# zdebruine/RcppML

Measured on AMD Instinct MI355X. Metric: ALS updates/sec (cols solved/s), k=64 sparse NMF, higher is better.
Workload: dtype f32; 1 GPU; configs[1]: simulateNMF 20000x100000 (x1 GPUs, column shards) 1%-dense CSC, k=64, MSE, coordinate-descent NNLS (cd_maxit=100, cd_tol=1e-8), L1 row normalisation, loss every iteration; rows=20000, cols_per_gpu=100000, nnz_per_gpu=20054852, k=64, solver=cd, cd_variant=auto, parallelism=column-shard x1

## Files before the change

rcppml_amd/csrc/kernels.hip.h:

```cpp
#pragma once
#include <hip/hip_runtime.h>
#include <stdint.h>

namespace rk {

#define RK_WAVE_SYNC()                                              \
    do {                                                            \
        __builtin_amdgcn_fence(__ATOMIC_RELEASE, "wavefront");      \
        __builtin_amdgcn_wave_barrier();                            \
        __builtin_amdgcn_fence(__ATOMIC_ACQUIRE, "wavefront");      \
    } while (0)

typedef float f32x4 __attribute__((ext_vector_type(4)));
typedef float f32x16 __attribute__((ext_vector_type(16)));
typedef double f64x4 __attribute__((ext_vector_type(4)));
typedef double f64x2 __attribute__((ext_vector_type(2)));

__device__ __forceinline__ float tabs(float v) { return __builtin_fabsf(v); }
__device__ __forceinline__ double tabs(double v) { return __builtin_fabs(v); }
__device__ __forceinline__ float tfma(float a, float b, float c) { return __builtin_fmaf(a, b, c); }
__device__ __forceinline__ double tfma(double a, double b, double c) { return __builtin_fma(a, b, c); }

__device__ __forceinline__ float sweep_quotient(float b, float , float ginv) { return b * ginv; }
__device__ __forceinline__ double sweep_quotient(double b, double gd, double ) { return b / gd; }
__device__ __forceinline__ double cd_quotient(double b, double gd, double ginv) {
    const double q0 = b * ginv;
    return __builtin_fma(__builtin_fma(-q0, gd, b), ginv, q0);
}
__device__ __forceinline__ float cd_quotient(float b, float , float ginv) { return b * ginv; }
__device__ __forceinline__ float cd_static_diff(float b, float , float ginv, float nl1) { return __builtin_fmaf(b, ginv, nl1); }
__device__ __forceinline__ double cd_static_diff(double b, double gd, double ginv, double nl1) { return cd_quotient(b, gd, ginv) + nl1; }
__device__ __forceinline__ float lane_value(float v, int i) {
    return __uint_as_float(__builtin_amdgcn_readlane(__float_as_uint(v), i));
}
__device__ __forceinline__ double lane_value(double v, int i) {
    const unsigned long long u = __double_as_longlong(v);
    const unsigned lo = __builtin_amdgcn_readlane((unsigned)u, i), hi = __builtin_amdgcn_readlane((unsigned)(u >> 32), i);
    return __longlong_as_double(((unsigned long long)hi << 32) | lo);
}

template <int B, int E, class Fn> __device__ __forceinline__ void cd_static_for(Fn&& fn) {
    if constexpr (B < E) { fn(std::integral_constant<int, B>{}); cd_static_for<B + 1, E>(fn); }
}
template <int I> __device__ __forceinline__ float cd_write_lane(float v, float value) {
    asm volatile("s_nop 1\n\tv_writelane_b32 %0, %1, %2" : "+v"(v) : "s"(value), "n"(I));
    return v;
}
template <int I> __device__ __forceinline__ double cd_write_lane(double v, double value) {
    unsigned long long u = __double_as_longlong(v);
    const unsigned long long w = __double_as_longlong(value);
    unsigned lo = (unsigned)u, hi = (unsigned)(u >> 32);
    asm volatile("s_nop 1\n\tv_writelane_b32 %0, %2, %4\n\tv_writelane_b32 %1, %3, %4" : "+v"(lo), "+v"(hi) : "s"((unsigned)w), "s"((unsigned)(w >> 32)), "n"(I));
    return __longlong_as_double(((unsigned long long)hi << 32) | lo);
}
__device__ __forceinline__ float cd_static_max(float a, float b, float inf) { return __builtin_amdgcn_fmed3f(a, b, inf); }
__device__ __forceinline__ double cd_static_max(double a, double b, double) { return __builtin_fmax(a, b); }
template <class T, int KP, class GC>
__device__ __forceinline__ T cd_static_one_sweep(T& b, T xe, T gd, T ginv, T nl1, T inf_rt, GC&& gcol) {
    T aown = T(0);
    cd_static_for<0, KP>([&](auto IC) {
        constexpr int i = decltype(IC)::value;
        const T diff = cd_static_diff(b, gd, ginv, nl1);
        const T ad = cd_static_max(diff, -xe, inf_rt);
        const T ad_i = lane_value(ad, i);
        b = tfma(-gcol(IC), ad_i, b);
        aown = cd_write_lane<i>(aown, ad_i);
    });
    return aown;
}
template <class T, int KP, class GC>
__device__ __forceinline__ int cd_static_sweeps(T& b, T& x, T gd, bool fok, T l1, int nonneg, int maxit, GC&& gcol) {
    const bool alive = fok && gd > T(0);
    const T ginv = alive ? T(1) / gd : T(0);
    const T nl1 = alive ? -l1 : T(0);
    const T pinf = static_cast<T>(__builtin_inff());
    const T inf_rt = maxit >= 0 ? pinf : T(0);
    for (int it = 0; it < maxit; ++it) {
        const T xe = !alive ? T(0) : (nonneg ? x : pinf);
        const T aown = cd_static_one_sweep<T, KP>(b, xe, gd, ginv, nl1, inf_rt, gcol);
        const T xn = x + aown;
        const bool moved = xn != x;
        x = xn;
        if (!__any(moved)) return it + 1;
    }
    return maxit > 0 ? maxit : 0;
}
template <class T, int KP, class GC>
__device__ __forceinline__ int cd_static_sweeps_tol(T& b, T& x, T gd, bool fok, int nonneg, int maxit, T tol, int k, GC&& gcol) {
    const bool alive = fok && gd > T(0);
    const T ginv = alive ? T(1) / gd : T(0);
    const T pinf = static_cast<T>(__builtin_inff());
    const T inf_rt = maxit >= 0 ? pinf : T(0);
    const bool check = tol > T(0);
    const T inv_k = T(1) / static_cast<T>(k);
    for (int it = 0; it < maxit; ++it) {
        const T xe = !alive ? T(0) : (nonneg ? x : pinf);
        const T aown = cd_static_one_sweep<T, KP>(b, xe, gd, ginv, T(0), inf_rt, gcol);
        const T xn = x + aown;
        const bool moved = xn != x;
        x = xn;
        if (check) {
            T term = fok ? (aown < T(0) ? -aown : aown) / ((x < T(0) ? -x : x) + T(1e-15)) : T(0);
#pragma unroll
            for (int off = 32; off > 0; off >>= 1) term += __shfl_xor(term, off, 64);
            if (term * inv_k < tol) return it + 1;
        } else if (!__any(moved)) return maxit;
    }
    return maxit;
}
template <int KP>
__device__ __forceinline__ int cd_static_sweeps_scaled_f32(float b, float& x, float gd, bool fok, float l1, int nonneg, int maxit,
                                                           float (&gcol)[KP]) {
    const bool alive = fok && gd > 0.f;
    const float ginv = alive ? 1.f / gd : 0.f;
    const float pinf = __builtin_inff();
    const float inf_rt = maxit >= 0 ? pinf : 0.f;
#pragma unroll
    for (int i = 0; i < KP; ++i) gcol[i] *= ginv;
    float d = __builtin_fmaf(b, ginv, alive ? -l1 : 0.f);
    for (int it = 0; it < maxit; ++it) {
        const float xe = nonneg ? x : pinf;
        float aown = 0.f;
        cd_static_for<0, KP>([&](auto IC) {
            constexpr int i = decltype(IC)::value;
            const float ad = cd_static_max(d, -xe, inf_rt);
            const float ad_i = lane_value(ad, i);
            d = __builtin_fmaf(-gcol[i], ad_i, d);
            aown = cd_write_lane<i>(aown, ad_i);
        });
        const float xn = x + aown;
        const bool moved = xn != x;
        x = xn;
        if (!__any(moved)) return it + 1;
    }
    return maxit > 0 ? maxit : 0;
}
template <int KP, class GC>
__device__ __forceinline__ int cd_static_sweeps_f32(float& b, float& x, float gd, bool fok, float l1, int nonneg, int maxit, GC&& gcol) {
    return cd_static_sweeps<float, KP>(b, x, gd, fok, l1, nonneg, maxit, gcol);
}

__device__ __forceinline__ float shfl_xor_t(float v, int m) { return __shfl_xor(v, m, 64); }
__device__ __forceinline__ double shfl_xor_t(double v, int m) { return __shfl_xor(v, m, 64); }

template <class T, int VEC> struct VecT;
template <> struct VecT<float, 1> { typedef float type; };
template <> struct VecT<float, 2> { typedef float type __attribute__((ext_vector_type(2))); };
template <> struct VecT<float, 4> { typedef float type __attribute__((ext_vector_type(4))); };
template <> struct VecT<double, 1> { typedef double type; };
template <> struct VecT<double, 2> { typedef double type __attribute__((ext_vector_type(2))); };

template <int T_TILES, bool VL, int STEPS>
__global__ __launch_bounds__(256) void gram_partial_f32(const float* __restrict__ F, int k, int64_t r,
                                                         float* __restrict__ partial) {
    constexpr int KP = 32 * T_TILES;
    __shared__ float red[3][T_TILES * 1024];
    const int ti = blockIdx.y;
    const int wave = threadIdx.x >> 6, lane = threadIdx.x & 63;
    const int64_t nw = (int64_t)gridDim.x * 4, wid = (int64_t)blockIdx.x * 4 + wave;
    const int64_t npairs = (r + 1) / 2;
    const int64_t per = (npairs + nw - 1) / nw;
    const int64_t p0 = wid * per;
    const int64_t p1 = p0 + per < npairs ? p0 + per : npairs;
    const int kk = lane >> 5, row = lane & 31;
    f32x16 acc[T_TILES];
#pragma unroll
    for (int t = 0; t < T_TILES; ++t)
#pragma unroll
        for (int v = 0; v < 16; ++v) acc[t][v] = 0.f;
    for (int64_t pb = p0; pb < p1; pb += STEPS) {
        float a[STEPS][T_TILES];
#pragma unroll
        for (int s = 0; s < STEPS; ++s) {
            const int64_t c = 2 * (pb + s) + kk;
            const bool cok = (pb + s) < p1 && c < r;
            const float* fc = F + c * (int64_t)k;
            if constexpr (VL) {
                typedef typename VecT<float, T_TILES>::type V;
                const int r0 = T_TILES * row;
                if (cok && r0 < k) {
                    const V v = *reinterpret_cast<const V*>(fc + r0);
#pragma unroll
                    for (int t = 0; t < T_TILES; ++t) a[s][t] = v[t];
                } else {
#pragma unroll
                    for (int t = 0; t < T_TILES; ++t) a[s][t] = 0.f;
                }
            } else {
#pragma unroll
                for (int t = 0; t < T_TILES; ++t) {
                    const int rr = 32 * t + row;
                    a[s][t] = (cok && rr < k) ? fc[rr] : 0.f;
                }
            }
        }
#pragma unroll
        for (int s = 0; s < STEPS; ++s)
#pragma unroll
            for (int t = 0; t < T_TILES; ++t) {
                float ai = a[s][0];
#pragma unroll
                for (int t2 = 1; t2 < T_TILES; ++t2) ai = (ti == t2) ? a[s][t2] : ai;
                acc[t] = __builtin_amdgcn_mfma_f32_32x32x2f32(ai, a[s][t], acc[t], 0, 0, 0);
            }
    }
    if (wave > 0) {
#pragma unroll
        for (int t = 0; t < T_TILES; ++t)
#pragma unroll
            for (int v = 0; v < 16; ++v) red[wave - 1][t * 1024 + v * 64 + lane] = acc[t][v];
    }
    __syncthreads();
    if (wave == 0) {
        float* out = partial + ((int64_t)blockIdx.x * KP * KP);
#pragma unroll
        for (int t = 0; t < T_TILES; ++t)
#pragma unroll
            for (int v = 0; v < 16; ++v) {
                float s = acc[t][v];
                s += red[0][t * 1024 + v * 64 + lane];
                s += red[1][t * 1024 + v * 64 + lane];
                s += red[2][t * 1024 + v * 64 + lane];
                const int is = (v & 3) + 8 * (v >> 2) + 4 * (lane >> 5), js = lane & 31;
                const int i = VL ? T_TILES * is + ti : 32 * ti + is;
                const int j = VL ? T_TILES * js + t : 32 * t + js;
                out[(int64_t)j * KP + i] = s;
            }
    }
}

template <int STEPS, bool SCALE>
__device__ __forceinline__ void gram_partial_f32_k64_body(float* __restrict__ F, int k, int64_t r, float* __restrict__ partial,
                                                          const unsigned bid, const unsigned nb, const float* __restrict__ sums,
                                                          int norm_type) {
    constexpr int KP = 64;
    __shared__ float red[3][4 * 1024];
    const int wave = threadIdx.x >> 6, lane = threadIdx.x & 63;
    const int64_t nw = (int64_t)nb * 4, wid = (int64_t)bid * 4 + wave;
    const int64_t npairs = (r + 1) / 2;
    const int64_t per = (npairs + nw - 1) / nw;
    const int64_t p0 = wid * per;
    const int64_t p1 = p0 + per < npairs ? p0 + per : npairs;
    const int kk = lane >> 5, row = lane & 31;
    f32x16 acc[2][2];
#pragma unroll
    for (int a = 0; a < 2; ++a)
#pragma unroll
        for (int b = 0; b < 2; ++b)
#pragma unroll
            for (int v = 0; v < 16; ++v) acc[a][b][v] = 0.f;
    typedef VecT<float, 2>::type V;
    float dv0 = 1.f, dv1 = 1.f;
    if constexpr (SCALE) {
        if (2 * row < k) {
            float s0 = sums[2 * row], s1 = sums[2 * row + 1];
            if (norm_type == 1) { s0 = sqrtf(s0); s1 = sqrtf(s1); }
            dv0 = s0 + 1e-15f; dv1 = s1 + 1e-15f;
        }
    }
    for (int64_t pb = p0; pb < p1; pb += STEPS) {
        float a[STEPS][2];
#pragma unroll
        for (int s = 0; s < STEPS; ++s) {
            const int64_t c = 2 * (pb + s) + kk;
            const bool cok = (pb + s) < p1 && c < r;
            const int r0 = 2 * row;
            if (cok && r0 < k) {
                V v = *reinterpret_cast<const V*>(F + c * (int64_t)k + r0);
                if constexpr (SCALE) {
                    v[0] = v[0] / dv0; v[1] = v[1] / dv1;
                    *reinterpret_cast<V*>(F + c * (int64_t)k + r0) = v;
                }
                a[s][0] = v[0]; a[s][1] = v[1];
            } else { a[s][0] = 0.f; a[s][1] = 0.f; }
        }
#pragma unroll
        for (int s = 0; s < STEPS; ++s)
#pragma unroll
            for (int ti = 0; ti < 2; ++ti)
#pragma unroll
                for (int t = 0; t < 2; ++t)
                    acc[ti][t] = __builtin_amdgcn_mfma_f32_32x32x2f32(a[s][ti], a[s][t], acc[ti][t], 0, 0, 0);
    }
    if (wave > 0) {
#pragma unroll
        for (int ti = 0; ti < 2; ++ti)
#pragma unroll
            for (int t = 0; t < 2; ++t)
#pragma unroll
                for (int v = 0; v < 16; ++v) red[wave - 1][(ti * 2 + t) * 1024 + v * 64 + lane] = acc[ti][t][v];
    }
    __syncthreads();
    if (wave == 0) {
        float* out = partial + ((int64_t)bid * KP * KP);
#pragma unroll
        for (int ti = 0; ti < 2; ++ti)
#pragma unroll
            for (int t = 0; t < 2; ++t)
#pragma unroll
                for (int v = 0; v < 16; ++v) {
                    float s = acc[ti][t][v];
                    s += red[0][(ti * 2 + t) * 1024 + v * 64 + lane];
                    s += red[1][(ti * 2 + t) * 1024 + v * 64 + lane];
                    s += red[2][(ti * 2 + t) * 1024 + v * 64 + lane];
                    const int is = (v & 3) + 8 * (v >> 2) + 4 * (lane >> 5), js = lane & 31;
                    out[(int64_t)(2 * js + t) * KP + (2 * is + ti)] = s;
                }
    }
}
template <int STEPS>
__global__ __launch_bounds__(256) void gram_partial_f32_k64(const float* __restrict__ F, int k, int64_t r,
                                                             float* __restrict__ partial) {
    gram_partial_f32_k64_body<STEPS, false>(const_cast<float*>(F), k, r, partial, blockIdx.x, gridDim.x, nullptr, 0);
}

template <int T_TILES>
__global__ __launch_bounds__(256) void gram_partial_f64(const double* __restrict__ F, int k, int64_t r,
                                                         double* __restrict__ partial) {
    constexpr int KP = 16 * T_TILES;
    __shared__ double red[3][T_TILES * 256];
    const int ti = blockIdx.y;
    const int wave = threadIdx.x >> 6, lane = threadIdx.x & 63;
    const int64_t nw = (int64_t)gridDim.x * 4, wid = (int64_t)blockIdx.x * 4 + wave;
    const int64_t nquad = (r + 3) / 4;
    const int64_t per = (nquad + nw - 1) / nw;
    const int64_t p0 = wid * per;
    const int64_t p1 = p0 + per < nquad ? p0 + per : nquad;
    const int kk = lane >> 4, row = lane & 15;
    f64x4 acc[T_TILES];
#pragma unroll
    for (int t = 0; t < T_TILES; ++t)
#pragma unroll
        for (int v = 0; v < 4; ++v) acc[t][v] = 0.0;
    const int rowi = 16 * ti + row;
#pragma unroll 2
    for (int64_t p = p0; p < p1; ++p) {
        const int64_t c = 4 * p + kk;
        const bool cok = c < r;
        const double* fc = F + c * (int64_t)k;
        const double ai = (cok && rowi < k) ? fc[rowi] : 0.0;
        double a[T_TILES];
#pragma unroll
        for (int t = 0; t < T_TILES; ++t) {
            const int rr = 16 * t + row;
            a[t] = (cok && rr < k) ? fc[rr] : 0.0;
        }
#pragma unroll
        for (int t = 0; t < T_TILES; ++t)
            acc[t] = __builtin_amdgcn_mfma_f64_16x16x4f64(ai, a[t], acc[t], 0, 0, 0);
    }
    if (wave > 0) {
#pragma unroll
        for (int t = 0; t < T_TILES; ++t)
#pragma unroll
            for (int v = 0; v < 4; ++v) red[wave - 1][t * 256 + v * 64 + lane] = acc[t][v];
    }
    __syncthreads();
    if (wave == 0) {
        double* out = partial + ((int64_t)blockIdx.x * KP * KP);
#pragma unroll
        for (int t = 0; t < T_TILES; ++t)
#pragma unroll
            for (int v = 0; v < 4; ++v) {
                double s = acc[t][v];
                s += red[0][t * 256 + v * 64 + lane];
                s += red[1][t * 256 + v * 64 + lane];
                s += red[2][t * 256 + v * 64 + lane];
                const int i = 16 * ti + (lane >> 4) + 4 * v;
                const int j = 16 * t + (lane & 15);
                out[(int64_t)j * KP + i] = s;
            }
    }
}

template <class T>
__device__ __forceinline__ void gram_finalize_body(const T* __restrict__ partial, int nblk, int KP, int k, T eps, T l2,
                                                   T* __restrict__ G, const unsigned bid) {
    const int e = bid * 8 + (threadIdx.x >> 5);
    const int sl = threadIdx.x & 31;
    T s = 0;
    if (e < KP * KP)
        for (int b = sl; b < nblk; b += 32) s += partial[(int64_t)b * KP * KP + e];
#pragma unroll
    for (int off = 16; off > 0; off >>= 1) s += shfl_xor_t(s, off);
    if (e >= KP * KP || sl != 0) return;
    const int i = e % KP, j = e / KP;
    if (i >= k || j >= k) return;
    if (i == j) { s += eps; s += l2; }
    G[(int64_t)j * k + i] = s;
}
template <class T>
__global__ __launch_bounds__(256) void gram_finalize(const T* __restrict__ partial, int nblk, int KP, int k, T eps, T l2,
                                                      T* __restrict__ G) {
    gram_finalize_body<T>(partial, nblk, KP, k, eps, l2, G, blockIdx.x);
}

template <class T, int VEC, int LPN, int U, bool NT>
__global__ __launch_bounds__(256) void rhs_kernel(const int* __restrict__ colptr,
                                                   const int* __restrict__ rowidx,
                                                   const T* __restrict__ vals, int64_t ncols,
                                                   const T* __restrict__ F, int k,
                                                   T* __restrict__ B) {
    constexpr int NG = 64 / LPN;
    const int64_t j = (int64_t)blockIdx.x * 4 + (threadIdx.x >> 6);
    if (j >= ncols) return;
    const int lane = threadIdx.x & 63;
    const int g = lane / LPN, li = lane % LPN;
    const int f0 = li * VEC;
    const bool fok = f0 < k;
    const int start = colptr[j], end = colptr[j + 1];
    T acc[VEC];
#pragma unroll
    for (int e = 0; e < VEC; ++e) acc[e] = T(0);
    const T* Fl = F + f0;
    for (int t = start + g; t < end; t += NG * U) {
        int rr[U];
        T vv[U];
#pragma unroll
        for (int u = 0; u < U; ++u) {
            const int tt = t + u * NG;
            const bool ok = tt < end;
            rr[u] = ok ? rowidx[tt] : 0;
            vv[u] = ok ? vals[tt] : T(0);
        }
        T ff[U][VEC];
#pragma unroll
        for (int u = 0; u < U; ++u) {
            if (fok) {
                const T* src = Fl + (int64_t)rr[u] * k;
                if constexpr (VEC == 1) {
                    ff[u][0] = src[0];
                } else {
                    typedef typename VecT<T, VEC>::type V;
                    V v;
                    if constexpr (NT) v = __builtin_nontemporal_load(reinterpret_cast<const V*>(src));
                    else v = *reinterpret_cast<const V*>(src);
#pragma unroll
                    for (int e = 0; e < VEC; ++e) ff[u][e] = v[e];
                }
            } else {
#pragma unroll
                for (int e = 0; e < VEC; ++e) ff[u][e] = T(0);
            }
        }
#pragma unroll
        for (int u = 0; u < U; ++u)
#pragma unroll
            for (int e = 0; e < VEC; ++e) acc[e] = tfma(vv[u], ff[u][e], acc[e]);
    }
#pragma unroll
    for (int off = LPN; off < 64; off <<= 1)
#pragma unroll
        for (int e = 0; e < VEC; ++e) acc[e] += shfl_xor_t(acc[e], off);
    if (g == 0 && fok) {
        T* dst = B + j * (int64_t)k + f0;
        if constexpr (VEC == 1) {
            dst[0] = acc[0];
        } else {
            typedef typename VecT<T, VEC>::type V;
            V v;
#pragma unroll
            for (int e = 0; e < VEC; ++e) v[e] = acc[e];
            *reinterpret_cast<V*>(dst) = v;
        }
    }
}

template <class T, int EPL>
__global__ __launch_bounds__(256) void rhs_generic_kernel(const int* __restrict__ colptr, const int* __restrict__ rowidx,
                                                           const T* __restrict__ vals, int64_t ncols,
                                                           const T* __restrict__ F, int k, T* __restrict__ B) {
    const int64_t j = (int64_t)blockIdx.x * 4 + (threadIdx.x >> 6);
    if (j >= ncols) return;
    const int lane = threadIdx.x & 63;
    T acc[EPL];
#pragma unroll
    for (int e = 0; e < EPL; ++e) acc[e] = T(0);
    const int start = colptr[j], end = colptr[j + 1];
#pragma unroll 4
    for (int t = start; t < end; ++t) {
        const int row = rowidx[t];
        const T v = vals[t];
        const T* src = F + (int64_t)row * k;
#pragma unroll
        for (int e = 0; e < EPL; ++e) {
            const int f = lane + 64 * e;
            if (f < k) acc[e] = tfma(v, src[f], acc[e]);
        }
    }
#pragma unroll
    for (int e = 0; e < EPL; ++e) {
        const int f = lane + 64 * e;
        if (f < k) B[j * (int64_t)k + f] = acc[e];
    }
}

template <class T, int VEC, int LPN, int U>
__global__ __launch_bounds__(256) void rhs_stage_kernel(const int* __restrict__ colptr,
                                                         const int* __restrict__ rowidx,
                                                         const T* __restrict__ vals, int64_t ncols,
                                                         const T* __restrict__ F, int k,
                                                         T* __restrict__ B) {
    constexpr int NG = 64 / LPN;
    constexpr int CH = NG * U;
    static_assert(CH <= 64, "one lane per staged nonzero");
    const int64_t j = (int64_t)blockIdx.x * 4 + (threadIdx.x >> 6);
    if (j >= ncols) return;
    const int lane = threadIdx.x & 63;
    const int g = lane / LPN, li = lane % LPN;
    const int f0 = li * VEC;
    const bool fok = f0 < k;
    const int start = colptr[j], end = colptr[j + 1];
    T acc[VEC];
#pragma unroll
    for (int e = 0; e < VEC; ++e) acc[e] = T(0);
    const T* Fl = F + (fok ? f0 : 0);
    int ri_n = 0;
    T vi_n = T(0);
    if (start < end) {
        const int tt = start + lane;
        const int tc = tt < end ? tt : end - 1;
        const int r0 = rowidx[tc];
        const T v0 = vals[tc];
        const bool ok = lane < CH && tt < end;
        ri_n = ok ? r0 : 0;
        vi_n = ok ? v0 : T(0);
    }
    for (int t0 = start; t0 < end; t0 += CH) {
        const int ri = ri_n;
        const T vi = vi_n;
        {
            const int tt = t0 + CH + lane;
            const int tc = tt < end ? tt : end - 1;
            const int r0 = rowidx[tc];
            const T v0 = vals[tc];
            __builtin_amdgcn_sched_barrier(0);
            const bool ok = lane < CH && tt < end;
            ri_n = ok ? r0 : 0;
            vi_n = ok ? v0 : T(0);
        }
        T ff[U][VEC];
        T vv[U];
#pragma unroll
        for (int u = 0; u < U; ++u) {
            const int nz = u * NG + g;
            const int r = __shfl(ri, nz, 64);
            vv[u] = __shfl(vi, nz, 64);
            const T* src = Fl + (int64_t)r * k;
            if constexpr (VEC == 1) {
                ff[u][0] = src[0];
            } else {
                typedef typename VecT<T, VEC>::type V;
                const V v = *reinterpret_cast<const V*>(src);
#pragma unroll
                for (int e = 0; e < VEC; ++e) ff[u][e] = v[e];
            }
        }
#pragma unroll
        for (int u = 0; u < U; ++u)
#pragma unroll
            for (int e = 0; e < VEC; ++e) acc[e] = tfma(vv[u], ff[u][e], acc[e]);
    }
#pragma unroll
    for (int off = LPN; off < 64; off <<= 1)
#pragma unroll
        for (int e = 0; e < VEC; ++e) acc[e] += shfl_xor_t(acc[e], off);
    if (g == 0 && fok) {
        T* dst = B + j * (int64_t)k + f0;
        if constexpr (VEC == 1) {
            dst[0] = acc[0];
        } else {
            typedef typename VecT<T, VEC>::type V;
            V v;
#pragma unroll
            for (int e = 0; e < VEC; ++e) v[e] = acc[e];
            *reinterpret_cast<V*>(dst) = v;
        }
    }
}

template <class T, int EPL, int U>
__global__ __launch_bounds__(256) void rhs_wave_kernel(const int* __restrict__ colptr,
                                                        const int* __restrict__ rowidx,
                                                        const T* __restrict__ vals, int64_t ncols,
                                                        const T* __restrict__ F, int k, T* __restrict__ B) {
    const int64_t j = __builtin_amdgcn_readfirstlane((int)((int64_t)blockIdx.x * 4 + (threadIdx.x >> 6)));
    if (j >= ncols) return;
    const int lane = threadIdx.x & 63;
    const bool fok = lane * EPL < k;
    const int f0 = fok ? lane * EPL : 0;
    const int start = colptr[j], end = colptr[j + 1];
    T acc[EPL];
#pragma unroll
    for (int e = 0; e < EPL; ++e) acc[e] = T(0);
    const T* Fl = F + f0;
    auto gather_fma = [&](const int (&rr)[U], const T (&vv)[U]) {
        T ff[U][EPL];
#pragma unroll
        for (int u = 0; u < U; ++u) {
            const T* src = Fl + (int64_t)rr[u] * k;
            if constexpr (EPL == 1) ff[u][0] = src[0];
            else {
                typedef typename VecT<T, EPL>::type V;
                const V v = *reinterpret_cast<const V*>(src);
#pragma unroll
                for (int e = 0; e < EPL; ++e) ff[u][e] = v[e];
            }
        }
#pragma unroll
        for (int u = 0; u < U; ++u)
#pragma unroll
            for (int e = 0; e < EPL; ++e) acc[e] = tfma(vv[u], ff[u][e], acc[e]);
    };
    struct __attribute__((packed, aligned(4))) IdxPack { int v[U]; };
// ... 1118 lines not shown
```

rcppml_amd/csrc/kernels_tail.hip.h:

```cpp
#pragma once
#include "kernels.hip.h"

namespace rk {

template <class T, int VEC>
__global__ __launch_bounds__(256) void tail_norm_hist_kernel(const T* __restrict__ X, int k, int64_t ncols, int norm_type,
                                                              T* __restrict__ partial, unsigned nb_norm, const int* __restrict__ sweeps,
                                                              unsigned int* __restrict__ part, unsigned nb_order) {
    if (blockIdx.x < nb_order) { order_hist_body(sweeps, ncols, part, blockIdx.x, nb_order); return; }
    const unsigned bid = blockIdx.x - nb_order;
    if constexpr (VEC > 0) row_norm_partial_vec_body<T, VEC>(X, k, ncols, norm_type, partial, bid, nb_norm);
    else row_norm_partial_body<T>(X, k, ncols, norm_type, partial, bid, nb_norm);
}
template <class T, int VEC>
__global__ __launch_bounds__(256) void tail_scale_scatter_kernel(T* __restrict__ X, int k, int64_t total, const T* __restrict__ sums,
                                                                  int norm_type, T* __restrict__ d, unsigned nb_scale,
                                                                  const int* __restrict__ sweeps, int64_t ncols,
                                                                  const unsigned int* __restrict__ part, int* __restrict__ order,
                                                                  unsigned nb_order) {
    if (blockIdx.x < nb_order) { order_scatter_body(sweeps, ncols, part, order, blockIdx.x, nb_order); return; }
    const unsigned bid = blockIdx.x - nb_order;
    if constexpr (VEC > 0) scale_rows_from_sums_vec_body<T, VEC>(X, k, total, sums, norm_type, d, bid, nb_scale);
    else scale_rows_from_sums_body<T>(X, k, total, sums, norm_type, d, bid, nb_scale);
}
template <int STEPS>
__global__ __launch_bounds__(256) void tail_scale_gram_k64_kernel(float* __restrict__ X, int k, int64_t ncols, const float* __restrict__ sums,
                                                                   int norm_type, float* __restrict__ d, float* __restrict__ gpartial,
                                                                   unsigned nb_gram, const int* __restrict__ sweeps,
                                                                   const unsigned int* __restrict__ part, int* __restrict__ order,
                                                                   unsigned nb_order) {
    if (blockIdx.x < nb_order) { order_scatter_body(sweeps, ncols, part, order, blockIdx.x, nb_order); return; }
    const unsigned bid = blockIdx.x - nb_order;
    if (bid == 0)
        for (int f = threadIdx.x; f < k; f += blockDim.x) {
            float s = sums[f];
            if (norm_type == 1) s = sqrtf(s);
            d[f] = s + 1e-15f;
        }
    gram_partial_f32_k64_body<STEPS, true>(X, k, ncols, gpartial, bid, nb_gram, sums, norm_type);
}
template <class T>
__global__ __launch_bounds__(256) void tail_gramfin_cross_kernel(const T* __restrict__ gpartial, int nblk_g, int KP, int k, T eps, T l2,
                                                                  T* __restrict__ G, const T* __restrict__ W, const T* __restrict__ Bw,
                                                                  const T* __restrict__ d, int64_t total, double* __restrict__ cpartial,
                                                                  unsigned nb_cross) {
    __shared__ double sh[4];
    if (blockIdx.x < nb_cross) cross_partial_body<T>(W, Bw, d, k, total, cpartial, blockIdx.x, nb_cross, sh);
    else gram_finalize_body<T>(gpartial, nblk_g, KP, k, eps, l2, G, blockIdx.x - nb_cross);
}

}
```

Before: 112.0 million cols/s.

## Software-pipeline k64 Gram partial loads with multi-stage register prefetch

```diff
diff --git a/rcppml_amd/csrc/kernels.hip.h b/rcppml_amd/csrc/kernels.hip.h
--- a/rcppml_amd/csrc/kernels.hip.h
+++ b/rcppml_amd/csrc/kernels.hip.h
@@ -235,7 +235,7 @@
                                                           int norm_type) {
     constexpr int KP = 64;
     __shared__ float red[3][4 * 1024];
-    const int wave = threadIdx.x >> 6, lane = threadIdx.x & 63;
+    const int wave = __builtin_amdgcn_readfirstlane((int)(threadIdx.x >> 6)), lane = threadIdx.x & 63;
     const int64_t nw = (int64_t)nb * 4, wid = (int64_t)bid * 4 + wave;
     const int64_t npairs = (r + 1) / 2;
     const int64_t per = (npairs + nw - 1) / nw;
@@ -250,37 +250,81 @@
 #pragma unroll
             for (int v = 0; v < 16; ++v) acc[a][b][v] = 0.f;
     typedef VecT<float, 2>::type V;
+    constexpr int DEPTH = 4;
+    const int r0 = 2 * row;
+    const bool rok = r0 < k;
+    const unsigned loff = (unsigned)(kk * k + r0);
+    int64_t pf = p1 > p0 ? p0 + (p1 - p0) / STEPS * STEPS : p0;
+    if (pf > p0 && 2 * pf > r) pf -= STEPS;
+    auto in_range = [&](const int64_t p) { return rok && p < p1 && 2 * p + kk < r; };
+    auto load_full = [&](V (&b)[STEPS], const int64_t pb) {
+#pragma unroll
+        for (int s = 0; s < STEPS; ++s) { b[s][0] = 0.f; b[s][1] = 0.f; }
+        if (rok) {
+#pragma unroll
+            for (int s = 0; s < STEPS; ++s) b[s] = *reinterpret_cast<const V*>(F + 2 * (pb + s) * (int64_t)k + loff);
+        }
+    };
+    auto mma_round = [&](const V (&v)[STEPS]) {
+#pragma unroll
+        for (int s = 0; s < STEPS; ++s)
+#pragma unroll
+            for (int ti = 0; ti < 2; ++ti)
+#pragma unroll
+                for (int t = 0; t < 2; ++t)
+                    acc[ti][t] = __builtin_amdgcn_mfma_f32_32x32x2f32(v[s][ti], v[s][t], acc[ti][t], 0, 0, 0);
+    };
+    V buf[DEPTH][STEPS], rag[STEPS];
+#pragma unroll
+    for (int j = 0; j < DEPTH; ++j)
+        if (p0 + j * STEPS < pf) load_full(buf[j], p0 + j * STEPS);
+    if (pf < p1) {
+#pragma unroll
+        for (int s = 0; s < STEPS; ++s) {
+            rag[s][0] = 0.f; rag[s][1] = 0.f;
+            if (in_range(pf + s)) rag[s] = *reinterpret_cast<const V*>(F + 2 * (pf + s) * (int64_t)k + loff);
+        }
+    }
     float dv0 = 1.f, dv1 = 1.f;
     if constexpr (SCALE) {
-        if (2 * row < k) {
+        if (rok) {
             float s0 = sums[2 * row], s1 = sums[2 * row + 1];
             if (norm_type == 1) { s0 = sqrtf(s0); s1 = sqrtf(s1); }
             dv0 = s0 + 1e-15f; dv1 = s1 + 1e-15f;
         }
     }
-    for (int64_t pb = p0; pb < p1; pb += STEPS) {
-        float a[STEPS][2];
-#pragma unroll
-        for (int s = 0; s < STEPS; ++s) {
-            const int64_t c = 2 * (pb + s) + kk;
-            const bool cok = (pb + s) < p1 && c < r;
-            const int r0 = 2 * row;
-            if (cok && r0 < k) {
-                V v = *reinterpret_cast<const V*>(F + c * (int64_t)k + r0);
+    for (int64_t pg = p0; pg < pf; pg += DEPTH * STEPS) {
+#pragma unroll
+        for (int j = 0; j < DEPTH; ++j) {
+            const int64_t pb = pg + j * STEPS;
+            if (pb < pf) {
+                V v[STEPS];
+#pragma unroll
+                for (int s = 0; s < STEPS; ++s) v[s] = buf[j][s];
+                if (pb + DEPTH * STEPS < pf) load_full(buf[j], pb + DEPTH * STEPS);
                 if constexpr (SCALE) {
-                    v[0] = v[0] / dv0; v[1] = v[1] / dv1;
-                    *reinterpret_cast<V*>(F + c * (int64_t)k + r0) = v;
+                    if (rok) {
+#pragma unroll
+                        for (int s = 0; s < STEPS; ++s) {
+                            v[s][0] = v[s][0] / dv0; v[s][1] = v[s][1] / dv1;
+                            *reinterpret_cast<V*>(F + 2 * (pb + s) * (int64_t)k + loff) = v[s];
+                        }
+                    }
                 }
-                a[s][0] = v[0]; a[s][1] = v[1];
-            } else { a[s][0] = 0.f; a[s][1] = 0.f; }
-        }
-#pragma unroll
-        for (int s = 0; s < STEPS; ++s)
-#pragma unroll
-            for (int ti = 0; ti < 2; ++ti)
-#pragma unroll
-                for (int t = 0; t < 2; ++t)
-                    acc[ti][t] = __builtin_amdgcn_mfma_f32_32x32x2f32(a[s][ti], a[s][t], acc[ti][t], 0, 0, 0);
+                mma_round(v);
+            }
+        }
+    }
+    if (pf < p1) {
+        if constexpr (SCALE) {
+#pragma unroll
+            for (int s = 0; s < STEPS; ++s)
+                if (in_range(pf + s)) {
+                    rag[s][0] = rag[s][0] / dv0; rag[s][1] = rag[s][1] / dv1;
+                    *reinterpret_cast<V*>(F + 2 * (pf + s) * (int64_t)k + loff) = rag[s];
+                }
+        }
+        mma_round(rag);
     }
     if (wave > 0) {
 #pragma unroll
@@ -309,7 +353,7 @@
     }
 }
 template <int STEPS>
-__global__ __launch_bounds__(256) void gram_partial_f32_k64(const float* __restrict__ F, int k, int64_t r,
+__global__ __launch_bounds__(256) __attribute__((amdgpu_waves_per_eu(2))) void gram_partial_f32_k64(const float* __restrict__ F, int k, int64_t r,
                                                              float* __restrict__ partial) {
     gram_partial_f32_k64_body<STEPS, false>(const_cast<float*>(F), k, r, partial, blockIdx.x, gridDim.x, nullptr, 0);
 }
diff --git a/rcppml_amd/csrc/kernels_tail.hip.h b/rcppml_amd/csrc/kernels_tail.hip.h
--- a/rcppml_amd/csrc/kernels_tail.hip.h
+++ b/rcppml_amd/csrc/kernels_tail.hip.h
@@ -24,7 +24,8 @@
     else scale_rows_from_sums_body<T>(X, k, total, sums, norm_type, d, bid, nb_scale);
 }
 template <int STEPS>
-__global__ __launch_bounds__(256) void tail_scale_gram_k64_kernel(float* __restrict__ X, int k, int64_t ncols, const float* __restrict__ sums,
+__global__ __launch_bounds__(256) __attribute__((amdgpu_waves_per_eu(2))) void tail_scale_gram_k64_kernel(
+                                                                   float* __restrict__ X, int k, int64_t ncols, const float* __restrict__ sums,
                                                                    int norm_type, float* __restrict__ d, float* __restrict__ gpartial,
                                                                    unsigned nb_gram, const int* __restrict__ sweeps,
                                                                    const unsigned int* __restrict__ part, int* __restrict__ order,
```

After: 112.5 million cols/s (median of 2 runs). No clear change (+0.4%).
